# lajoiepy/cslam

Hardware: AMD Instinct MI355X
Metric: keyframes/sec (extract+match) on 100kx4096-D bank (higher is better)
Workload: dtype f32

## Files before the change

### cslam_amd/_lib.py

```python
import ctypes as C
import os
import subprocess

_HERE = os.path.dirname(os.path.abspath(__file__))
LIB_PATH = os.environ.get("CSLAM_HIP_LIB") or os.path.join(_HERE, "libcslam_hip.so")
CSRC_DIR = os.path.join(_HERE, "csrc")

F32, F64 = 0, 1
MODE_AUTO, MODE_SCAN, MODE_MFMA = 0, 1, 2


class CslamHipError(RuntimeError):
    pass


class CslamGraphError(CslamHipError):
    """CSLAM_E_GRAPH: the graph admits no Fiedler pair (not connected, singular junction Laplacian, TraceMIN breakdown) --
    the condition under which the reference's networkx call raises and acm.py:436-466 re-draws its start point.  Not a
    failure of the GPU path."""


class CslamUnsupportedError(CslamHipError):
    """CSLAM_E_UNSUPPORTED: an optional run-time dependency (RCCL, rocBLAS / rocSOLVER) was not found on this host."""

# ... 129 lines not shown
                                                   _vp, _vp, _vp, _vp, _vp, _vp, _vp, _vp, _vp, _vp, _vp, _vp, _vp, _vp, _vp, _vp, _vp, _vp]),
    "cslam_stereo_dense_dev": (_i, [_vp, _vp, _vp, _vp, _i, _vp, _i, _i, _i, _i, _vp, _vp, _vp, _vp, _vp, _vp, _vp, _vp]),
    "cslam_cloud_keyframes_stereo_dev": (_i, [_vp, _vp, _i, _vp, _vp, _vp, _vp, _vp, _i, _i, _i, _i, _i, C.c_double, C.c_double,
                                              _vp, _vp, _vp, _vp, _vp, _vp, _vp, _vp, _vp, _vp, _vp]),
    "cslam_wino4_fused_c64_h_dev": (_i, [_vp, _vp, _vp, _vp, _i, _i, _i, _i, _i, _i, _vp, C.c_float, _vp, _vp, _vp]),
    "cslam_conv3x3_direct_h_dev": (_i, [_vp, _vp, _vp, _i, _i, _i, _i, _i, _i, _i, _vp, _f, _vp, _vp, _vp]),
    "cslam_conv3x3_direct_r_dev": (_i, [_vp, _vp, _vp, _i, _i, _i, _i, _i, _i, _i, _vp, C.c_float, _vp, _vp, _vp]),
    "cslam_conv3x3_direct_r2_dev": (_i, [_vp, _vp, _vp, _i, _i, _i, _i, _i, _i, _i, _vp, C.c_float, _vp, _vp, _vp]),
    "cslam_conv_stem_direct_h_dev": (_i, [_vp, _vp, _vp, _vp, C.c_float, _vp, _vp, C.c_float, _i, _i, _i, _i, _vp, _vp, _vp, _vp]),
    "cslam_wino4_stem_c64_h_dev": (_i, [_vp, _vp, _vp, _vp, C.c_float, _vp, _vp, _i, _i, _i, _i, _vp, C.c_float, _vp, _vp, _vp]),
    "cslam_debug_wfh_prof_dev": (_i, [_vp]),
    "cslam_conv3x3_c3_amax_dev": (_i, [_vp, _vp, _vp, _i, _i, _i, _i, _i, _vp, _vp, _vp]),
    "cslam_wino4_input_h2_dev": (_i, [_vp, _i, _i, _i, _i, _vp, _vp, _vp]),
    "cslam_wino_gemm_h2_dev": (_i, [_vp, _vp, _i64, _i, _i, _vp, _vp]),
    "cslam_wino4_chain_h2_dev": (_i, [_vp, _vp, _i, _i, _i, _i, _vp, C.c_float, _vp, C.c_float, C.c_float, _vp, _vp, _vp, _vp]),
    "cslam_wino_zgemm_h2_dev": (_i, [_vp, _vp, _i64, _i, _i, _vp, _vp]),
    "cslam_wino4_output_z_dev": (_i, [_vp, _vp, _i, _i, _i, _i, _i, _i, _vp, C.c_float, _vp, _vp, _vp]),
    "cslam_conv_igemm_h2_dev": (_i, [_vp, _vp, _vp, _vp, _i, _i, _i, _i, _i, _i, _i, _i, _i, _i, _vp, C.c_float, _vp, _vp, _vp]),
    "cslam_conv_stem_pool_igemm_h2_dev": (_i, [_vp, _vp, _vp, _i, _i, _i, _i, _i, _i, _i, _i, _vp, C.c_float, _vp, _vp, _vp]),
    "cslam_conv_igemm_h2p_dev": (_i, [_vp, _i, _vp, _vp, _vp, _vp, _i, _vp, _i, _i, _i, _i, _i, _i, _i, _i, _i, _i, _vp, C.c_float,
                                      C.c_float, C.c_float, _vp, _i, _vp, _vp, _vp]),
    "cslam_conv3x3_direct_r_pairs_dev": (_i, [_vp, _vp, _vp, _i, _i, _i, _i, _i, _vp, C.c_float, C.c_float, C.c_float, _vp, _vp, _vp, _vp]),
    "cslam_conv3x3_direct_hp_dev": (_i, [_vp, _vp, _vp, _vp, _i, _i, _i, _i, _i, _i, _i, C.c_float, _vp, _vp, _vp]),
    "cslam_conv3x3_direct_p_dev": (_i, [_vp, _i, _vp, _vp, _vp, _vp, _i, _vp, _i, _i, _i, _i, _i, _i, _vp, C.c_float, C.c_float, C.c_float,
                                        _vp, _i, _vp, _vp, _vp]),
    "cslam_comm_unique_id": (_i, [_vp]),
    "cslam_comm_init": (_i, [_i, _i, _vp, _i, C.POINTER(_vp)]),
    "cslam_comm_destroy": (_i, [_vp]),
    "cslam_comm_info": (_i, [_vp, C.POINTER(_i), C.POINTER(_i)]),
    "cslam_allgather_queries_dev": (_i, [_vp, _vp, _i64, _i64, _vp, _vp]),
# ... 73 lines not shown
```

### cslam_amd/csrc/wino_chain.hip

```cpp
#include "common.h"
#include "pairs.h"
#include <hip/hip_fp16.h>

typedef float cf4 __attribute__((ext_vector_type(4)));
typedef unsigned cu2 __attribute__((ext_vector_type(2)));
typedef unsigned cu4 __attribute__((ext_vector_type(4)));

__device__ __forceinline__ void wc_at4(const cf4 m0, const cf4 m1, const cf4 m2, const cf4 m3, const cf4 m4, const cf4 m5,
                                       cf4 &s0, cf4 &s1, cf4 &s2, cf4 &s3) {
    const cf4 a = m1 + m2, bq = m1 - m2, c = m3 + m4, e = m3 - m4;
    s0 = m0 + a + c;
    s1 = bq + 2.0f * e;
    s2 = a + 4.0f * c;
    s3 = bq + 8.0f * e + m5;
}
__device__ __forceinline__ void wc_bt4(cf4 &d0, cf4 &d1, cf4 &d2, cf4 &d3, cf4 &d4, cf4 &d5) {
    const cf4 r0 = 4.0f * d0 - 5.0f * d2 + d4;
    const cf4 r1 = -4.0f * (d1 + d2) + d3 + d4;
    const cf4 r2 = 4.0f * (d1 - d2) - d3 + d4;
    const cf4 r3 = 2.0f * (d3 - d1) - d2 + d4;
    const cf4 r4 = 2.0f * (d1 - d3) - d2 + d4;
    const cf4 r5 = 4.0f * d1 - 5.0f * d3 + d5;
    d0 = r0; d1 = r1; d2 = r2; d3 = r3; d4 = r4; d5 = r5;
}

#define WC_THREADS 128
#define WC_RING 9

struct WcArgs {
    const float *mb;
    __half *vb;
    unsigned moff, voff;
    float *rp;
    int64_t mplane, vplane, mrow, vrow;
    int H, TH, Wr, tj;
    float inv, sc;
    cf4 bv;
    cf4 clim;
    bool odd;
};

template <int CG, bool OUT, bool LOAD, bool IN>
__device__ __forceinline__ void wc_step(const WcArgs &a, const int r, cf4 (&m)[36], float &vmax) {
    if (OUT) {
        cf4 s[4][6];
#pragma unroll
        for (int j = 0; j < 6; ++j)
            wc_at4(m[j], m[6 + j], m[12 + j], m[18 + j], m[24 + j], m[30 + j], s[0][j], s[1][j], s[2][j], s[3][j]);
#pragma unroll
        for (int i = 0; i < 4; ++i) {
            cf4 o[4];
            wc_at4(s[i][0], s[i][1], s[i][2], s[i][3], s[i][4], s[i][5], o[0], o[1], o[2], o[3]);
            const int h = 4 * r + i;
            float *row = a.rp + ((h % WC_RING) * a.Wr + 4 * a.tj) * CG;
            const cf4 lim = h < a.H ? a.clim : (cf4)(0.0f);
#pragma unroll
            for (int j = 0; j < 4; ++j) {
                cf4 v = __builtin_elementwise_max(o[j] * a.inv + a.bv, (cf4)(0.0f));
                v = __builtin_elementwise_min(v, (cf4)(lim[j]));
                vmax = fmaxf(fmaxf(vmax, fmaxf(v.x, v.y)), fmaxf(v.z, v.w));
                *(cf4 *)(row + j * CG) = v;
            }
        }
    }
    __syncthreads();
    if (LOAD) {
        const float *p = a.mb + (r + 1) * a.mrow;
#pragma unroll
        for (int q = 0; q < 36; ++q) m[q] = __builtin_nontemporal_load((const cf4 *)(p + q * a.mplane + a.moff));
    }
    if (IN) {
        const int h0 = 4 * (r - 1) - 1, w0 = 4 * a.tj - 1;
        const int Hr = 4 * a.TH;
        cf4 d[6][6];
#pragma unroll
        for (int i = 0; i < 6; ++i) {
            const int hh = h0 + i;
            const float *row = a.rp + ((hh + WC_RING) % WC_RING) * a.Wr * CG;
#pragma unroll
            for (int j = 0; j < 6; ++j) {
                const int ww = w0 + j;
                const bool in = (hh >= 0) & (hh < Hr) & (ww >= 0) & (ww < a.Wr);
                cf4 v = *(const cf4 *)(row + (j == 0 ? max(ww, 0) : j == 5 ? min(ww, a.Wr - 1) : ww) * CG);
                asm("" : "+v"(v));
                d[i][j] = in ? v * a.sc : (cf4)(0.0f);
            }
        }
#pragma unroll
        for (int j = 0; j < 6; ++j) wc_bt4(d[0][j], d[1][j], d[2][j], d[3][j], d[4][j], d[5][j]);
#pragma unroll
        for (int i = 0; i < 6; ++i) wc_bt4(d[i][0], d[i][1], d[i][2], d[i][3], d[i][4], d[i][5]);
        __half *o = a.vb + (r - 1) * a.vrow;
#pragma unroll
        for (int i = 0; i < 6; ++i)
#pragma unroll
            for (int j = 0; j < 6; ++j) {
                const cf4 v = d[i][j];
                const __half2 h0v = __floats2half2_rn(v.x, v.y), h1v = __floats2half2_rn(v.z, v.w);
                const __half2 l0v = __floats2half2_rn(sub_half<0>(v.x, h0v), sub_half<1>(v.y, h0v));
                const __half2 l1v = __floats2half2_rn(sub_half<0>(v.z, h1v), sub_half<1>(v.w, h1v));
                cu2 hi, lo;
                hi.x = *(const unsigned *)&h0v; hi.y = *(const unsigned *)&h1v;
                lo.x = *(const unsigned *)&l0v; lo.y = *(const unsigned *)&l1v;
                const cu2 give = a.odd ? hi : lo;
                cu2 got;
                got.x = (unsigned)__builtin_amdgcn_mov_dpp((int)give.x, 0xB1, 0xF, 0xF, true);
                got.y = (unsigned)__builtin_amdgcn_mov_dpp((int)give.y, 0xB1, 0xF, 0xF, true);
                cu4 v16;
                if (a.odd) { v16.x = got.x; v16.y = got.y; v16.z = lo.x; v16.w = lo.y; }
                else { v16.x = hi.x; v16.y = hi.y; v16.z = got.x; v16.w = got.y; }
                __builtin_nontemporal_store(v16, (cu4 *)(o + (6 * i + j) * a.vplane + a.voff));
            }
    }
    __syncthreads();
}

template <int CG>
__global__ __launch_bounds__(WC_THREADS) void wino4_chain_h2_kernel(const float *__restrict__ M, const float *__restrict__ bias,
                                                                     int B, int H, int W, int C,
                                                                     const unsigned *__restrict__ vscale, float inv_su,
                                                                     const unsigned *__restrict__ amax_x, float wl1, float bmax,
                                                                     unsigned *__restrict__ amax_out,
                                                                     unsigned *__restrict__ bound_out, __half *__restrict__ V2) {
    extern __shared__ __attribute__((aligned(16))) float ring[];
    __shared__ unsigned wg_amax;
    constexpr int C4G = CG / 4;
    WcArgs a;
    a.H = H;
    a.TH = (H + 3) >> 2;
    const int TW = (W + 3) >> 2;
    a.Wr = 4 * TW;
    const int ncg = C / CG;
    const int b = blockIdx.x / ncg, cg = blockIdx.x - b * ncg;
    a.tj = threadIdx.x / C4G;
    const int c4 = threadIdx.x % C4G;
    const int c = cg * CG + 4 * c4;
    const int64_t T = (int64_t)B * a.TH * TW;
    const int64_t t0 = (int64_t)b * a.TH * TW;
    if (threadIdx.x == 0) wg_amax = 0u;

    a.inv = inv_su / scale_le_327_68(__uint_as_float(*vscale));
    const float bound = fmaf(__uint_as_float(*amax_x), wl1, bmax);
    a.sc = scale_le_327_68(bound);
    if (blockIdx.x == 0 && threadIdx.x == 0) *bound_out = __float_as_uint(bound);
    a.bv = bias ? *(const cf4 *)(bias + c) : (cf4)(0.0f);
#pragma unroll
    for (int j = 0; j < 4; ++j) a.clim[j] = 4 * a.tj + j < W ? __builtin_inff() : 0.0f;
    a.odd = threadIdx.x & 1;
    a.mplane = T * C;
    a.vplane = T * 2 * C;
    a.mrow = (int64_t)TW * C;
    a.vrow = (int64_t)TW * 2 * C;
    a.mb = M + t0 * C + cg * CG;
    a.vb = V2 + t0 * 2 * C + cg * 2 * CG;
    a.moff = a.tj * C + 4 * c4;
    a.voff = a.tj * 2 * C + (c4 >> 3) * 64 + (4 * c4 & 31) + (a.odd ? 32 - 4 : 0);
    a.rp = ring + 4 * c4;
    float vmax = 0.0f;

    cf4 m[36];
#pragma unroll
    for (int q = 0; q < 36; ++q) m[q] = __builtin_nontemporal_load((const cf4 *)(a.mb + q * a.mplane + a.moff));
    const int TH = a.TH;
    if (TH == 1) {
        wc_step<CG, true, false, false>(a, 0, m, vmax);
    } else {
        wc_step<CG, true, true, false>(a, 0, m, vmax);
#pragma unroll 1
        for (int r = 1; r < TH - 1; ++r) wc_step<CG, true, true, true>(a, r, m, vmax);
        wc_step<CG, true, false, true>(a, TH - 1, m, vmax);
    }
    wc_step<CG, false, false, true>(a, TH, m, vmax);
#pragma unroll
    for (int o = 32; o > 0; o >>= 1) vmax = fmaxf(vmax, __shfl_xor(vmax, o, 64));
    if ((threadIdx.x & 63) == 0) atomicMax(&wg_amax, __float_as_uint(vmax));
    __syncthreads();
    if (threadIdx.x == 0 && wg_amax > *(volatile unsigned *)amax_out) atomicMax(amax_out, wg_amax);
}

template <int CG>
static int wino4_chain_launch(const float *d_M, const float *d_bias, int B, int H, int W, int C, const unsigned *d_vscale,
                              float inv_su, const unsigned *d_amax_x, float wl1, float bmax, unsigned *d_amax_out,
                              unsigned *d_bound_out, void *d_V2, void *stream) {
    const size_t lds = (size_t)WC_RING * 4 * ((W + 3) / 4) * CG * sizeof(float);
    ARG_CHECK(lds <= 144 * 1024, "map too wide for the LDS ring");
    static DeviceOnce once;
    int dev;
    if (once.todo(&dev)) {
        HIP_TRY(hipFuncSetAttribute((const void *)wino4_chain_h2_kernel<CG>, hipFuncAttributeMaxDynamicSharedMemorySize, 144 * 1024));
        once.done(dev);
    }
    hipLaunchKernelGGL(wino4_chain_h2_kernel<CG>, dim3((unsigned)((int64_t)B * (C / CG))), dim3(((W + 3) / 4) * (CG / 4)), lds, (hipStream_t)stream,
                       d_M, d_bias, B, H, W, C, d_vscale, inv_su, d_amax_x, wl1, bmax, d_amax_out, d_bound_out, (__half *)d_V2);
    HIP_TRY(hipGetLastError());
    return CSLAM_OK;
}

CSLAM_API int cslam_wino4_chain_h2_dev(const float *d_M, const float *d_bias, int B, int H, int W, int C,
                                       const unsigned *d_vscale, float inv_su, const unsigned *d_amax_x, float wl1, float bmax,
                                       unsigned *d_amax_out, unsigned *d_bound_out, void *d_V2, void *stream) {
    PTR_DEVICE(d_M);
    ARG_CHECK(d_M && d_V2 && d_vscale && d_amax_x && d_amax_out && d_bound_out, "NULL argument");
    ARG_CHECK(B >= 1 && H >= 1 && W >= 1, "empty map");
    ARG_CHECK(C >= 32 && (C % 32) == 0, "C must be a multiple of 32");
    ARG_CHECK(inv_su > 0.0f && wl1 >= 0.0f && bmax >= 0.0f, "inv_su must be positive, wl1 and bmax non-negative");
    const int TW = (W + 3) / 4;
    ARG_CHECK(TW <= 16, "maps wider than 64 pixels stay on the separate transforms");
    ARG_CHECK((int64_t)B * (C / 32) < (1LL << 31), "too many frames for one launch");
    if (TW <= 4 && (C % 128) == 0)
        return wino4_chain_launch<128>(d_M, d_bias, B, H, W, C, d_vscale, inv_su, d_amax_x, wl1, bmax, d_amax_out, d_bound_out, d_V2, stream);
    if (TW <= 8 && (C % 64) == 0)
        return wino4_chain_launch<64>(d_M, d_bias, B, H, W, C, d_vscale, inv_su, d_amax_x, wl1, bmax, d_amax_out, d_bound_out, d_V2, stream);
    return wino4_chain_launch<32>(d_M, d_bias, B, H, W, C, d_vscale, inv_su, d_amax_x, wl1, bmax, d_amax_out, d_bound_out, d_V2, stream);
}
```

### cslam_amd/vpr/netvlad.py

```python
import os
import pickle
from os.path import isfile, join

import numpy as np
import torch
from torch import nn

from .. import _lib
from . import heads
from .backbones import vgg16_features_trunk
from .winograd import WinogradTrunk

IMAGENET_DEFAULT_MEAN = heads.IMAGENET_DEFAULT_MEAN
IMAGENET_DEFAULT_STD = heads.IMAGENET_DEFAULT_STD


def _share_dir():
    try:
        from ament_index_python.packages import get_package_share_directory
        return get_package_share_directory("cslam")
    except Exception:
        return ""


def _strip_module(state):
    return {k.replace(".module.", "."): v for k, v in state.items()}
# ... 123 lines not shown
        self.trunk = None
        self._online = self._online_trunk = None
        self._lanes = []
        cent = torch.randn((64, 512), generator=g)
        cent = cent / cent.norm(dim=1, keepdim=True) * 0.5
        w = 2.0 * 10.0 * cent
        self.pool.load(w, cent)
        din = 64 * 512
        comp = torch.randn((pca_dim, din), generator=g, dtype=torch.float32) / din ** 0.5
        self.pca_components = heads.padded_rows(pca_dim, din, self.device)
        self.pca_components.copy_(comp)
        self.pca_pairs = heads.pca_pair_weights(self.pca_components)
        self.pca_mean_proj = torch.zeros(pca_dim, dtype=torch.float32, device=self.device)
        self.pca_inv_scale = None

    @torch.no_grad()
    def compute_embeddings_device(self, frames_u8, backbone_dtype=None, _trunk=None):
        x = heads.preprocess(frames_u8.contiguous(), self.crop)
        if self.backbone_conv == 'direct' or (backbone_dtype is not None and backbone_dtype != torch.float32):
            x = x.contiguous(memory_format=torch.channels_last)
        if backbone_dtype is not None and backbone_dtype != torch.float32:
            with torch.autocast("cuda", dtype=backbone_dtype):
                f = self.encoder(x)
            f = f.float()
        elif self.backbone_conv in ('winograd', 'winograd2'):
            if _trunk is not None:
                f = _trunk(x)
            else:
                if self.trunk is None:
                    self.trunk = WinogradTrunk(self.encoder, min_in_channels=64,
                                               tile=4 if self.backbone_conv == 'winograd' else 2, forms=self.trunk_forms)
                    self.trunk.input_bound = heads.normalised_image_bound()
                f = self.trunk(x)
        else:
            f = self.encoder(x)
        if heads.vlad_pairs_fit(f, self.pool.centroids, self.pca_pairs):
            a2, _ = heads.vlad_aggregate_pairs(f, self.pool.conv_weight, self.pool.conv_bias, self.pool.centroids,
                                               self.pca_pairs[0].shape[0], heads.VLAD_BOUND)
            return heads.pca_project_from_pairs(a2, self.pca_components, self.pca_mean_proj, self.pca_inv_scale, self.pca_pairs,
                                                heads.VLAD_BOUND)
        v = self.pool(f)
        return heads.pca_project(v, self.pca_components, self.pca_mean_proj, self.pca_inv_scale, self.pca_pairs, heads.VLAD_BOUND)

    def compute_embeddings_batch_device(self, frames_u8, chunk=512, lanes=2):
        if lanes <= 1 or frames_u8.shape[0] <= chunk or self.backbone_conv not in ('winograd', 'winograd2'):
            outs = [self.compute_embeddings_device(frames_u8[s:s + chunk]) for s in range(0, int(frames_u8.shape[0]), chunk)]
            return outs[0] if len(outs) == 1 else torch.cat(outs)

        def lane_trunk(i):
            if i == 0 and self.trunk is not None:
                return self.trunk
            trunk = WinogradTrunk(self.encoder, min_in_channels=64, tile=4 if self.backbone_conv == 'winograd' else 2, forms=self.trunk_forms)
            trunk.input_bound = heads.normalised_image_bound()
            if i == 0:
                self.trunk = trunk
            return trunk
        return heads.extract_over_lanes(self._lanes, frames_u8, chunk, lanes, lane_trunk,
                                        lambda fr, trunk: self.compute_embeddings_device(fr, _trunk=trunk))

    def compute_embedding(self, keyframe):
        if not self.enable:
            return np.random.rand(128)
        keyframe = np.ascontiguousarray(keyframe)
        if self.use_graph and keyframe.dtype == np.uint8 and keyframe.ndim == 3:
            if self._online is None:
                if self.backbone_conv != 'direct':
                    self._online_trunk = WinogradTrunk(self.encoder, min_in_channels=64, tile=2)
                self._online = heads.OnlineGraph(
# ... 7 lines not shown
```

### cslam_amd/vpr/winograd.py

```python
import os

import torch
from torch import nn

from .. import _lib
from .conv_kernels import (PairAct, _amax_slot, _out, _po, _residual_like, conv3x3_direct_h, conv3x3_direct_hp,
                           conv3x3_direct_p, conv3x3_direct_r, conv3x3_direct_r2, conv3x3_direct_r_pairs, conv_igemm, conv_igemm_p,
                           conv_stem_direct_h, direct_p_fits, pairs_to_float, stem_pool_fits, wino_fused64, wino_fused64_h,
                           wino_stem64_h)
from .heads import _p, _stream
from .pair_weights import (direct_pair_weights, direct_r2_pair_weights, direct_r_pair_weights, fused64_pair_weights,
                           fused64_weights, igemm_pair_weights, out_bound, split16_pair_weights, split16_weights,
                           stem_direct_pair_weights, stem_pair_weights, wino_weights)


def _pair(v):
    return tuple(v) if isinstance(v, (tuple, list)) else (v, v)


_TUNED = {"done": False}


def use_tuned_gemms():
    if _TUNED["done"] or os.environ.get("CSLAM_TUNED_GEMM", "1") == "0" or not torch.cuda.is_available():
# ... 24 lines not shown


def _f4_fits(B, H, W):
    t4h, t4w = -(-H // 4), -(-W // 4)
    return B * t4h * t4w >= 512 and 16 * t4h * t4w <= 1.35 * H * W


def _pair_pipeline(ws, x, layers, slots, relu, pool, residual, amax_out):
    lib = _lib.load()
    B, Cin, H, W = x.shape
    T = B * -(-H // 4) * -(-W // 4)
    s = _stream(x)
    V2 = ws._buf("V", 36 * T * Cin, x.device)
    _lib.check(lib.cslam_wino4_input_h2_dev(_p(x), B, H, W, Cin, _p(slots[0:1]), _p(V2), s))
    vscale = slots[0:1]
    for j, (U2, bias, wl1, bmax) in enumerate(layers):
        Cout = U2[0].shape[1]
        M = ws._buf("M", 36 * T * Cout, x.device)
        _lib.check(lib.cslam_wino_gemm_h2_dev(_p(V2), _p(U2[0]), T, Cin, Cout, _p(M), s))
        if j + 1 < len(layers):
            bound = ws._buf("chain_bounds", len(layers), x.device)[j + 1:j + 2]
            V2 = ws._buf("V", 36 * T * Cout, x.device)
            _lib.check(lib.cslam_wino4_chain_h2_dev(_p(M), _po(bias), B, H, W, Cout, _p(vscale), float(U2[1]), _p(slots[j:j + 1]),
                                                    wl1, bmax, _p(slots[j + 1:j + 2]), _p(bound), _p(V2), s))
            vscale, Cin = bound, Cout
    y = _out(B, Cout, H, W, pool, x.device)
    _lib.check(lib.cslam_wino4_output_scaled_dev(_p(M), _po(bias), _po(_residual_like(residual, y)), B, H, W, Cout, int(relu),
                                                 int(pool), _p(vscale), float(U2[1]), _po(amax_out), _p(y), s))
    return y


def wino_conv3x3(ws, x, U, U4, bias, relu, pool=False, residual=None, U3=None, amax_in=None, amax_out=None, U2=None):
    lib = _lib.load()
    B, Cin, H, W = x.shape
    Cout = U.shape[2]
    assert residual is None or not pool
    four = U4 is not None and _f4_fits(B, H, W)
    ws.amax_written = four and amax_out is not None
    T = B * -(-H // 4) * -(-W // 4) if four else B * -(-H // 2) * -(-W // 2)
    s = _stream(x)
    slot = None
    if four and (U2 is not None or U3 is not None):
        slot = amax_in if amax_in is not None else _amax_slot(x, ws._buf("amax", 1, x.device))
    z = four and U2 is not None and residual is None and _z_form(Cin, Cout)
    if four and U2 is not None and not z:
        return _pair_pipeline(ws, x, [(U2, bias, None, None)], slot, relu, pool, residual, amax_out)
    inv_su = 1.0
    if z:
        V2 = ws._buf("V", 36 * T * Cin, x.device)
        M = ws._buf("M", 36 * T * Cout, x.device)
        _lib.check(lib.cslam_wino4_input_h2_dev(_p(x), B, H, W, Cin, _p(slot), _p(V2), s))
        _lib.check(lib.cslam_wino_zgemm_h2_dev(_p(V2), _p(U2[0]), T, Cin, Cout, _p(M), s))
        inv_su = U2[1]
    elif slot is not None:
        V3 = ws._buf("V", (36 * T * 3 * Cin + 1) // 2, x.device).view(torch.float16)[:36 * T * 3 * Cin].view(36, T, 3 * Cin)
        _lib.check(lib.cslam_wino4_input_h3_dev(_p(x), B, H, W, Cin, _p(slot), _p(V3), s))
        M = torch.bmm(V3, U3[0], out_dtype=torch.float32)
        inv_su = U3[1]
    else:
        n2, Uu, fin = (36, U4, lib.cslam_wino4_input_dev) if four else (16, U, lib.cslam_wino_input_dev)
        V = ws._buf("V", n2 * T * Cin, x.device).view(n2, T, Cin)
# ... 164 lines not shown

class _Step(object):
    __slots__ = ("kind", "module", "conv", "relu", "pool", "U", "U4", "U3", "U2", "Up", "Uph", "bias", "stem", "Wd", "Wr", "Wdr", "Wdr2", "wl1", "bmax")

    def __init__(self):
        for name in self.__slots__:
            setattr(self, name, None)
        self.kind, self.relu, self.pool = "torch", False, False


def _wants(st):
    return st.U3 is not None or st.U2 is not None or st.Uph is not None or st.Wd is not None


TRUNK_FORMS = {"conv_direct": 1, "conv_direct_r": True, "conv_direct_r2": True, "stem_direct": True, "wino_stem": True, "fused_h": True, "split16_min_cin": None,
               "wino_chain": True}
CHAIN_TILE_COLS = (5, 16)
FP32_GEMM_FORMS = {"split16_min_cin": 0, "fused_h": False, "wino_stem": False}


def _pool2_at(mods, i):
    p = mods[i] if i < len(mods) else None
    return (isinstance(p, nn.MaxPool2d) and p.kernel_size in (2, (2, 2)) and p.stride in (2, (2, 2))
            and p.padding in (0, (0, 0)) and not p.ceil_mode)


class WinogradTrunk(_Workspace):

    def __init__(self, encoder, min_in_channels=256, tile=2, fused64=None, split16_h3=False, forms=None):
        super().__init__()
        self.encoder = encoder
# ... 72 lines not shown
                    st.pool = True
                    i += 1
            else:
                st.kind, st.module = "torch", m
                i += 1
            self.steps.append(st)
        if self.forms["wino_stem"]:
            for a, b in zip(self.steps, self.steps[1:]):
                if (a.kind == "c3" and a.relu and a.conv.out_channels == 64 and b.kind == "wino" and b.Uph is not None
                        and b.relu and b.conv.out_channels == 64):
                    a.stem = stem_pair_weights(a.conv.weight)
                    if self.forms["stem_direct"]:
                        a.Wr = stem_direct_pair_weights(b.conv.weight)
        return self

    def _chain_len(self, k, B, H, W):
        if not (self.forms["wino_chain"] and _f4_fits(B, H, W) and CHAIN_TILE_COLS[0] <= -(-W // 4) <= CHAIN_TILE_COLS[1]):
            return 1
        pair = lambda st_: (st_.kind == "wino" and st_.U2 is not None and st_.Wd is None and st_.Up is None
                            and not _z_form(st_.conv.in_channels, st_.conv.out_channels))
        n = 1
        while (k + n < len(self.steps) and pair(self.steps[k + n - 1]) and pair(self.steps[k + n])
               and self.steps[k + n - 1].relu and not self.steps[k + n - 1].pool):
            n += 1
        return n

    def _want(self, slots, j):
        return slots[j:j + 1] if j < len(self.steps) and _wants(self.steps[j]) else None


    def _stem_pair(self, k, x, slots):
        st, (B, _, H, W) = self.steps[k], x.shape
        nxt = self.steps[k + 1] if st.stem is not None else None
        if nxt is None or not (B * -(-H // 16) * -(-W // 16) >= self.fused_min_blocks and not (nxt.pool and (H % 2 or W % 2))
                               and B * H * W * 64 < 2 ** 31):
            return None
        slot = slots[k:k + 1]
        if self.input_bound is not None:
            slot.fill_(float(self.input_bound))
        else:
# ... 51 lines not shown
    def _fused64(self, k, x, have, slots):
        st, (B, _, H, W) = self.steps[k], x.shape
        if st.Up is None or (st.pool and (H % 2 or W % 2)):
            return None
        bh, bw = (16, 16) if st.Up.shape[1] == 36 else (8, 16)
        if B * -(-H // bh) * -(-W // bw) * st.Up.shape[2] // 4 < self.fused_min_blocks:
            return None
        if st.Uph is None or x.numel() >= 2 ** 31:
            return wino_fused64(x, st.Up, st.bias, st.relu, st.pool), None, 0
        slot = _amax_slot(x, slots[k:k + 1], have)
        want = self._want(slots, k + 1)
        return wino_fused64_h(x, st.Uph, st.bias, st.relu, st.pool, slot, want), want is not None, 0

    def _winograd(self, k, x, have, slots):
        st = self.steps[k]
        n = self._chain_len(k, x.shape[0], x.shape[2], x.shape[3])
        if n == 1:
            want = self._want(slots, k + 1)
            y = wino_conv3x3(self, x, st.U, st.U4, st.bias, st.relu, st.pool, U3=st.U3, U2=st.U2,
                             amax_in=slots[k:k + 1] if have else None, amax_out=want)
            return y, want is not None and self.amax_written, 0
        _amax_slot(x, slots[k:k + 1], have)
        want = self._want(slots, k + n)
        chain = self.steps[k:k + n]
        y = _pair_pipeline(self, x, [(t.U2, t.bias, t.wl1, t.bmax) for t in chain], slots[k:k + n], chain[-1].relu, chain[-1].pool,
                           None, want)
        return y, want is not None, n - 1

    @torch.no_grad()
    def __call__(self, x):
        slots = have = None
        if any(_wants(st) for st in self.steps):
            slots = self._buf("amax_slots", len(self.steps) + 1, x.device)
            slots.zero_()
        k = 0
        while k < len(self.steps):
            st = self.steps[k]
            if st.kind == "c3":
                x = x.contiguous()
                x, have, ran = self._stem_pair(k, x, slots) or self._first_layer(k, x, slots)
            else:
# ... 11 lines not shown
```

### include/cslam_hip.h

```cpp
#ifndef CSLAM_HIP_H
#define CSLAM_HIP_H

#include <stdint.h>

#ifdef __cplusplus
extern "C" {
#endif

#define CSLAM_OK 0
#define CSLAM_E_INVALID (-1)
#define CSLAM_E_HIP (-2)
#define CSLAM_E_NOMEM (-3)
#define CSLAM_E_DIM (-4)
#define CSLAM_E_UNSUPPORTED (-5)
#define CSLAM_E_GRAPH (-6)
#define CSLAM_E_LIMIT (-7)

#define CSLAM_F32 0
#define CSLAM_F64 1

#define CSLAM_MODE_AUTO 0
#define CSLAM_MODE_SCAN 1
#define CSLAM_MODE_MFMA 2

// ... 291 lines not shown
int cslam_wino_output_dev(const float *d_M, const float *d_bias, const float *d_residual, int B, int H, int W,
                          int C, int relu, int pool, float *d_y, void *stream);
int cslam_wino4_input_dev(const float *d_x, int B, int H, int W, int C, float *d_V, void *stream);
int cslam_wino4_output_dev(const float *d_M, const float *d_bias, const float *d_residual, int B, int H, int W,
                           int C, int relu, int pool, float *d_y, void *stream);
int cslam_absmax_dev(const float *d_x, int64_t n, unsigned *d_slot, void *stream);
int cslam_wino4_output_scaled_dev(const float *d_M, const float *d_bias, const float *d_residual, int B, int H, int W,
                                  int C, int relu, int pool, const unsigned *d_amax, float inv_su, unsigned *d_amax_out,
                                  float *d_y, void *stream);
int cslam_wino4_input_h2_dev(const float *d_x, int B, int H, int W, int C, const unsigned *d_amax, void *d_V2,
                             void *stream);
int cslam_wino_gemm_h2_dev(const void *d_V2, const void *d_U2, int64_t T, int Cin, int Cout, float *d_M, void *stream);
int cslam_wino4_chain_h2_dev(const float *d_M, const float *d_bias, int B, int H, int W, int C, const unsigned *d_vscale,
                             float inv_su, const unsigned *d_amax_x, float wl1, float bmax, unsigned *d_amax_out,
                             unsigned *d_bound_out, void *d_V2, void *stream);
int cslam_wino_zgemm_h2_dev(const void *d_V2, const void *d_U2, int64_t T, int Cin, int Cout, float *d_Z, void *stream);
int cslam_wino4_output_z_dev(const float *d_Z, const float *d_bias, int B, int H, int W, int C, int relu, int pool,
                             const unsigned *d_amax, float inv_su, unsigned *d_amax_out, float *d_y, void *stream);

int cslam_wino4_fused_c64_h_dev(const float *d_x, const void *d_Uh, const float *d_bias, const float *d_residual, int B,
                                int H, int W, int Cout, int relu, int pool, const unsigned *d_amax, float inv_su,
                                unsigned *d_amax_out, float *d_y, void *stream);
int cslam_conv3x3_direct_h_dev(const float *d_x, const void *d_w2, const float *d_bias, int B, int H, int W, int Cin, int Cout,
                               int relu, int pool, const unsigned *d_amax, float inv_sw, unsigned *d_amax_out, float *d_y,
                               void *stream);
int cslam_conv3x3_c3_amax_dev(const float *d_x, const float *d_wt, const float *d_bias, int B, int H, int W, int Cout,
                              int relu, float *d_y, unsigned *d_amax_out, void *stream);

int cslam_wino4_stem_c64_h_dev(const float *d_x0, const void *d_w1, const float *d_b1, const float *d_sumw, float inv_sw,
                               const void *d_Uh, const float *d_bias, int B, int H, int W, int pool,
// ... 64 lines not shown
```

Baseline: 18980.

## Add whole-map and pooled Winograd chain links to fuse more conv layers

Extends the fused Winograd output-to-input chain kernel with two new modes. A 'map' mode handles small feature maps (at most 16 tiles) in one block without the row-walk ring. A 'pool' mode applies a 2x2 max-pool inside the chain so the next layer's input transform is produced directly. The trunk planner now builds chains across these links, which removes separate output, pool and input-transform kernels and their HBM round trips. Map mode is on by default only for the extractor; pool mode is off by default, and the map kernel uses a different launch size and more LDS.

```diff
diff --git a/cslam_amd/_lib.py b/cslam_amd/_lib.py
--- a/cslam_amd/_lib.py
+++ b/cslam_amd/_lib.py
@@ -167,6 +167,8 @@
     "cslam_wino4_input_h2_dev": (_i, [_vp, _i, _i, _i, _i, _vp, _vp, _vp]),
     "cslam_wino_gemm_h2_dev": (_i, [_vp, _vp, _i64, _i, _i, _vp, _vp]),
     "cslam_wino4_chain_h2_dev": (_i, [_vp, _vp, _i, _i, _i, _i, _vp, C.c_float, _vp, C.c_float, C.c_float, _vp, _vp, _vp, _vp]),
+    "cslam_wino4_chain_map_h2_dev": (_i, [_vp, _vp, _i, _i, _i, _i, _vp, C.c_float, _vp, C.c_float, C.c_float, _vp, _vp, _vp, _i, _vp]),
+    "cslam_wino4_chain_pool_h2_dev": (_i, [_vp, _vp, _i, _i, _i, _i, _vp, C.c_float, _vp, C.c_float, C.c_float, _vp, _vp, _vp, _vp]),
     "cslam_wino_zgemm_h2_dev": (_i, [_vp, _vp, _i64, _i, _i, _vp, _vp]),
     "cslam_wino4_output_z_dev": (_i, [_vp, _vp, _i, _i, _i, _i, _i, _i, _vp, C.c_float, _vp, _vp, _vp]),
     "cslam_conv_igemm_h2_dev": (_i, [_vp, _vp, _vp, _vp, _i, _i, _i, _i, _i, _i, _i, _i, _i, _i, _vp, C.c_float, _vp, _vp, _vp]),
diff --git a/cslam_amd/csrc/wino_chain.hip b/cslam_amd/csrc/wino_chain.hip
--- a/cslam_amd/csrc/wino_chain.hip
+++ b/cslam_amd/csrc/wino_chain.hip
@@ -26,6 +26,10 @@
 
 #define WC_THREADS 128
 #define WC_RING 9
+#define WC_POOL_RING 8
+
+enum { WC_WALK, WC_MAP, WC_POOL };
+__host__ __device__ constexpr int wc_ring(int mode) { return mode == WC_WALK ? WC_RING : mode == WC_POOL ? WC_POOL_RING : 0; }
 
 struct WcArgs {
     const float *mb;
@@ -34,94 +38,108 @@
     float *rp;
     int64_t mplane, vplane, mrow, vrow;
     int H, TH, Wr, tj;
+    int TWn;
     float inv, sc;
     cf4 bv;
     cf4 clim;
     bool odd;
 };
 
-template <int CG, bool OUT, bool LOAD, bool IN>
+template <int CG, int MODE>
+__device__ __forceinline__ void wc_out(const WcArgs &a, const int r, const cf4 (&m)[36], float &vmax) {
+    constexpr int RING = wc_ring(MODE);
+    cf4 s[4][6];
+    cf4 top[4];
+#pragma unroll
+    for (int j = 0; j < 6; ++j)
+        wc_at4(m[j], m[6 + j], m[12 + j], m[18 + j], m[24 + j], m[30 + j], s[0][j], s[1][j], s[2][j], s[3][j]);
+#pragma unroll
+    for (int i = 0; i < 4; ++i) {
+        cf4 o[4];
+        wc_at4(s[i][0], s[i][1], s[i][2], s[i][3], s[i][4], s[i][5], o[0], o[1], o[2], o[3]);
+        const int h = 4 * r + i;
+        float *row = a.rp + ((RING ? h % RING : h) * a.Wr + 4 * a.tj) * CG;
+        const cf4 lim = h < a.H ? a.clim : (cf4)(0.0f);
+#pragma unroll
+        for (int j = 0; j < 4; ++j) {
+            cf4 v = __builtin_elementwise_max(o[j] * a.inv + a.bv, (cf4)(0.0f));
+            v = __builtin_elementwise_min(v, (cf4)(lim[j]));
+            vmax = fmaxf(fmaxf(vmax, fmaxf(v.x, v.y)), fmaxf(v.z, v.w));
+            if (MODE != WC_POOL) *(cf4 *)(row + j * CG) = v;
+            else top[j] = (i & 1) ? __builtin_elementwise_max(top[j], v) : v;
+        }
+        if (MODE == WC_POOL && (i & 1)) {
+            float *prow = a.rp + (((2 * r + (i >> 1)) % RING) * a.Wr + 2 * a.tj) * CG;
+            *(cf4 *)prow = __builtin_elementwise_max(top[0], top[1]);
+            *(cf4 *)(prow + CG) = __builtin_elementwise_max(top[2], top[3]);
+        }
+    }
+}
+
+template <int CG, int MODE>
+__device__ __forceinline__ void wc_in(const WcArgs &a, const int tr, __half *o) {
+    constexpr int RING = wc_ring(MODE);
+    const int h0 = 4 * tr - 1, w0 = 4 * a.tj - 1;
+    const int Hr = (MODE == WC_POOL ? 2 : 4) * a.TH;
+    cf4 d[6][6];
+#pragma unroll
+    for (int i = 0; i < 6; ++i) {
+        const int hh = h0 + i;
+        const float *row = a.rp + (RING ? (hh + RING) % RING : min(max(hh, 0), Hr - 1)) * a.Wr * CG;
+#pragma unroll
+        for (int j = 0; j < 6; ++j) {
+            const int ww = w0 + j;
+            const bool in = (hh >= 0) & (hh < Hr) & (ww >= 0) & (ww < a.Wr);
+            cf4 v = *(const cf4 *)(row + (j == 0 ? max(ww, 0) : j == 5 || MODE == WC_POOL ? min(ww, a.Wr - 1) : ww) * CG);
+            asm("" : "+v"(v));
+            d[i][j] = in ? v * a.sc : (cf4)(0.0f);
+        }
+    }
+#pragma unroll
+    for (int j = 0; j < 6; ++j) wc_bt4(d[0][j], d[1][j], d[2][j], d[3][j], d[4][j], d[5][j]);
+#pragma unroll
+    for (int i = 0; i < 6; ++i) wc_bt4(d[i][0], d[i][1], d[i][2], d[i][3], d[i][4], d[i][5]);
+#pragma unroll
+    for (int i = 0; i < 6; ++i)
+#pragma unroll
+        for (int j = 0; j < 6; ++j) {
+            const cf4 v = d[i][j];
+            const __half2 h0v = __floats2half2_rn(v.x, v.y), h1v = __floats2half2_rn(v.z, v.w);
+            const __half2 l0v = __floats2half2_rn(sub_half<0>(v.x, h0v), sub_half<1>(v.y, h0v));
+            const __half2 l1v = __floats2half2_rn(sub_half<0>(v.z, h1v), sub_half<1>(v.w, h1v));
+            cu2 hi, lo;
+            hi.x = *(const unsigned *)&h0v; hi.y = *(const unsigned *)&h1v;
+            lo.x = *(const unsigned *)&l0v; lo.y = *(const unsigned *)&l1v;
+            const cu2 give = a.odd ? hi : lo;
+            cu2 got;
+            got.x = (unsigned)__builtin_amdgcn_mov_dpp((int)give.x, 0xB1, 0xF, 0xF, true);
+            got.y = (unsigned)__builtin_amdgcn_mov_dpp((int)give.y, 0xB1, 0xF, 0xF, true);
+            cu4 v16;
+            if (a.odd) { v16.x = got.x; v16.y = got.y; v16.z = lo.x; v16.w = lo.y; }
+            else { v16.x = hi.x; v16.y = hi.y; v16.z = got.x; v16.w = got.y; }
+            __builtin_nontemporal_store(v16, (cu4 *)(o + (6 * i + j) * a.vplane + a.voff));
+        }
+}
+
+template <int CG, int MODE, bool OUT, bool LOAD, bool IN>
 __device__ __forceinline__ void wc_step(const WcArgs &a, const int r, cf4 (&m)[36], float &vmax) {
-    if (OUT) {
-        cf4 s[4][6];
-#pragma unroll
-        for (int j = 0; j < 6; ++j)
-            wc_at4(m[j], m[6 + j], m[12 + j], m[18 + j], m[24 + j], m[30 + j], s[0][j], s[1][j], s[2][j], s[3][j]);
-#pragma unroll
-        for (int i = 0; i < 4; ++i) {
-            cf4 o[4];
-            wc_at4(s[i][0], s[i][1], s[i][2], s[i][3], s[i][4], s[i][5], o[0], o[1], o[2], o[3]);
-            const int h = 4 * r + i;
-            float *row = a.rp + ((h % WC_RING) * a.Wr + 4 * a.tj) * CG;
-            const cf4 lim = h < a.H ? a.clim : (cf4)(0.0f);
-#pragma unroll
-            for (int j = 0; j < 4; ++j) {
-                cf4 v = __builtin_elementwise_max(o[j] * a.inv + a.bv, (cf4)(0.0f));
-                v = __builtin_elementwise_min(v, (cf4)(lim[j]));
-                vmax = fmaxf(fmaxf(vmax, fmaxf(v.x, v.y)), fmaxf(v.z, v.w));
-                *(cf4 *)(row + j * CG) = v;
-            }
-        }
-    }
+    if (OUT) wc_out<CG, MODE>(a, r, m, vmax);
     __syncthreads();
     if (LOAD) {
         const float *p = a.mb + (r + 1) * a.mrow;
 #pragma unroll
         for (int q = 0; q < 36; ++q) m[q] = __builtin_nontemporal_load((const cf4 *)(p + q * a.mplane + a.moff));
     }
-    if (IN) {
-        const int h0 = 4 * (r - 1) - 1, w0 = 4 * a.tj - 1;
-        const int Hr = 4 * a.TH;
-        cf4 d[6][6];
-#pragma unroll
-        for (int i = 0; i < 6; ++i) {
-            const int hh = h0 + i;
-            const float *row = a.rp + ((hh + WC_RING) % WC_RING) * a.Wr * CG;
-#pragma unroll
-            for (int j = 0; j < 6; ++j) {
-                const int ww = w0 + j;
-                const bool in = (hh >= 0) & (hh < Hr) & (ww >= 0) & (ww < a.Wr);
-                cf4 v = *(const cf4 *)(row + (j == 0 ? max(ww, 0) : j == 5 ? min(ww, a.Wr - 1) : ww) * CG);
-                asm("" : "+v"(v));
-                d[i][j] = in ? v * a.sc : (cf4)(0.0f);
-            }
-        }
-#pragma unroll
-        for (int j = 0; j < 6; ++j) wc_bt4(d[0][j], d[1][j], d[2][j], d[3][j], d[4][j], d[5][j]);
-#pragma unroll
-        for (int i = 0; i < 6; ++i) wc_bt4(d[i][0], d[i][1], d[i][2], d[i][3], d[i][4], d[i][5]);
-        __half *o = a.vb + (r - 1) * a.vrow;
-#pragma unroll
-        for (int i = 0; i < 6; ++i)
-#pragma unroll
-            for (int j = 0; j < 6; ++j) {
-                const cf4 v = d[i][j];
-                const __half2 h0v = __floats2half2_rn(v.x, v.y), h1v = __floats2half2_rn(v.z, v.w);
-                const __half2 l0v = __floats2half2_rn(sub_half<0>(v.x, h0v), sub_half<1>(v.y, h0v));
-                const __half2 l1v = __floats2half2_rn(sub_half<0>(v.z, h1v), sub_half<1>(v.w, h1v));
-                cu2 hi, lo;
-                hi.x = *(const unsigned *)&h0v; hi.y = *(const unsigned *)&h1v;
-                lo.x = *(const unsigned *)&l0v; lo.y = *(const unsigned *)&l1v;
-                const cu2 give = a.odd ? hi : lo;
-                cu2 got;
-                got.x = (unsigned)__builtin_amdgcn_mov_dpp((int)give.x, 0xB1, 0xF, 0xF, true);
-                got.y = (unsigned)__builtin_amdgcn_mov_dpp((int)give.y, 0xB1, 0xF, 0xF, true);
-                cu4 v16;
-                if (a.odd) { v16.x = got.x; v16.y = got.y; v16.z = lo.x; v16.w = lo.y; }
-                else { v16.x = hi.x; v16.y = hi.y; v16.z = got.x; v16.w = got.y; }
-                __builtin_nontemporal_store(v16, (cu4 *)(o + (6 * i + j) * a.vplane + a.voff));
-            }
-    }
+    if (IN && MODE != WC_POOL) wc_in<CG, MODE>(a, r - 1, a.vb + (r - 1) * a.vrow);
+    if (IN && MODE == WC_POOL && !(r & 1) && r >= 2 && a.tj < a.TWn) wc_in<CG, MODE>(a, (r >> 1) - 1, a.vb + ((r >> 1) - 1) * a.vrow);
     __syncthreads();
 }
 
-template <int CG>
-__global__ __launch_bounds__(WC_THREADS) void wino4_chain_h2_kernel(const float *__restrict__ M, const float *__restrict__ bias,
-                                                                     int B, int H, int W, int C,
-                                                                     const unsigned *__restrict__ vscale, float inv_su,
-                                                                     const unsigned *__restrict__ amax_x, float wl1, float bmax,
-                                                                     unsigned *__restrict__ amax_out,
-                                                                     unsigned *__restrict__ bound_out, __half *__restrict__ V2) {
+template <int CG, int MODE>
+__device__ __forceinline__ void wc_kernel(const float *__restrict__ M, const float *__restrict__ bias, int B, int H, int W, int C,
+                                          const unsigned *__restrict__ vscale, float inv_su, const unsigned *__restrict__ amax_x,
+                                          float wl1, float bmax, unsigned *__restrict__ amax_out, unsigned *__restrict__ bound_out,
+                                          __half *__restrict__ V2) {
     extern __shared__ __attribute__((aligned(16))) float ring[];
     __shared__ unsigned wg_amax;
     constexpr int C4G = CG / 4;
@@ -129,14 +147,18 @@
     a.H = H;
     a.TH = (H + 3) >> 2;
     const int TW = (W + 3) >> 2;
-    a.Wr = 4 * TW;
+    a.Wr = (MODE == WC_POOL ? 2 : 4) * TW;
+    const int THn = MODE == WC_POOL ? ((H >> 1) + 3) >> 2 : a.TH;
+    a.TWn = MODE == WC_POOL ? ((W >> 1) + 3) >> 2 : TW;
     const int ncg = C / CG;
     const int b = blockIdx.x / ncg, cg = blockIdx.x - b * ncg;
-    a.tj = threadIdx.x / C4G;
+    const int tile = threadIdx.x / C4G;
+    const int ti = MODE == WC_MAP ? tile / TW : 0;
+    a.tj = tile - ti * TW;
     const int c4 = threadIdx.x % C4G;
     const int c = cg * CG + 4 * c4;
-    const int64_t T = (int64_t)B * a.TH * TW;
-    const int64_t t0 = (int64_t)b * a.TH * TW;
+    const int64_t T = (int64_t)B * a.TH * TW, Tn = (int64_t)B * THn * a.TWn;
+    const int64_t t0 = (int64_t)b * a.TH * TW, t0n = (int64_t)b * THn * a.TWn;
     if (threadIdx.x == 0) wg_amax = 0u;
 
     a.inv = inv_su / scale_le_327_68(__uint_as_float(*vscale));
@@ -148,13 +170,13 @@
     for (int j = 0; j < 4; ++j) a.clim[j] = 4 * a.tj + j < W ? __builtin_inff() : 0.0f;
     a.odd = threadIdx.x & 1;
     a.mplane = T * C;
-    a.vplane = T * 2 * C;
+    a.vplane = Tn * 2 * C;
     a.mrow = (int64_t)TW * C;
-    a.vrow = (int64_t)TW * 2 * C;
+    a.vrow = (int64_t)a.TWn * 2 * C;
     a.mb = M + t0 * C + cg * CG;
-    a.vb = V2 + t0 * 2 * C + cg * 2 * CG;
-    a.moff = a.tj * C + 4 * c4;
-    a.voff = a.tj * 2 * C + (c4 >> 3) * 64 + (4 * c4 & 31) + (a.odd ? 32 - 4 : 0);
+    a.vb = V2 + t0n * 2 * C + cg * 2 * CG;
+    a.moff = tile * C + 4 * c4;
+    a.voff = tile * 2 * C + (c4 >> 3) * 64 + (4 * c4 & 31) + (a.odd ? 32 - 4 : 0);
     a.rp = ring + 4 * c4;
     float vmax = 0.0f;
 
@@ -162,15 +184,26 @@
 #pragma unroll
     for (int q = 0; q < 36; ++q) m[q] = __builtin_nontemporal_load((const cf4 *)(a.mb + q * a.mplane + a.moff));
     const int TH = a.TH;
-    if (TH == 1) {
-        wc_step<CG, true, false, false>(a, 0, m, vmax);
+    if (MODE == WC_MAP) {
+        wc_out<CG, MODE>(a, ti, m, vmax);
+        __syncthreads();
+        wc_in<CG, MODE>(a, ti, a.vb);
     } else {
-        wc_step<CG, true, true, false>(a, 0, m, vmax);
+        if (TH == 1) {
+            wc_step<CG, MODE, true, false, false>(a, 0, m, vmax);
+        } else {
+            wc_step<CG, MODE, true, true, false>(a, 0, m, vmax);
 #pragma unroll 1
-        for (int r = 1; r < TH - 1; ++r) wc_step<CG, true, true, true>(a, r, m, vmax);
-        wc_step<CG, true, false, true>(a, TH - 1, m, vmax);
-    }
-    wc_step<CG, false, false, true>(a, TH, m, vmax);
+            for (int r = 1; r < TH - 1; ++r) wc_step<CG, MODE, true, true, true>(a, r, m, vmax);
+            wc_step<CG, MODE, true, false, true>(a, TH - 1, m, vmax);
+        }
+        if (MODE == WC_WALK) {
+            wc_step<CG, MODE, false, false, true>(a, TH, m, vmax);
+        } else {
+#pragma unroll 1
+            for (int r = TH; r <= 2 * THn; ++r) wc_step<CG, MODE, false, false, true>(a, r, m, vmax);
+        }
+    }
 #pragma unroll
     for (int o = 32; o > 0; o >>= 1) vmax = fmaxf(vmax, __shfl_xor(vmax, o, 64));
     if ((threadIdx.x & 63) == 0) atomicMax(&wg_amax, __float_as_uint(vmax));
@@ -178,38 +211,84 @@
     if (threadIdx.x == 0 && wg_amax > *(volatile unsigned *)amax_out) atomicMax(amax_out, wg_amax);
 }
 
+#define WC_PARAMS const float *__restrict__ M, const float *__restrict__ bias, int B, int H, int W, int C,                                   \
+                  const unsigned *__restrict__ vscale, float inv_su, const unsigned *__restrict__ amax_x, float wl1, float bmax,           \
+                  unsigned *__restrict__ amax_out, unsigned *__restrict__ bound_out, __half *__restrict__ V2
+#define WC_PASS M, bias, B, H, W, C, vscale, inv_su, amax_x, wl1, bmax, amax_out, bound_out, V2
+
 template <int CG>
+__global__ __launch_bounds__(WC_THREADS) void wino4_chain_h2_kernel(WC_PARAMS) { wc_kernel<CG, WC_WALK>(WC_PASS); }
+
+template <int CG>
+__global__ __launch_bounds__(WC_THREADS) void wino4_chain_pool_h2_kernel(WC_PARAMS) { wc_kernel<CG, WC_POOL>(WC_PASS); }
+
+template <int CG>
+__global__ __launch_bounds__(4 * CG, 2) void wino4_chain_map_h2_kernel(WC_PARAMS) { wc_kernel<CG, WC_MAP>(WC_PASS); }
+
+template <int CG, int MODE>
 static int wino4_chain_launch(const float *d_M, const float *d_bias, int B, int H, int W, int C, const unsigned *d_vscale,
                               float inv_su, const unsigned *d_amax_x, float wl1, float bmax, unsigned *d_amax_out,
                               unsigned *d_bound_out, void *d_V2, void *stream) {
-    const size_t lds = (size_t)WC_RING * 4 * ((W + 3) / 4) * CG * sizeof(float);
+    const int TH = (H + 3) / 4, TW = (W + 3) / 4;
+    const size_t lds = (size_t)(MODE == WC_MAP ? 4 * TH : wc_ring(MODE)) * (MODE == WC_POOL ? 2 : 4) * TW * CG * sizeof(float);
     ARG_CHECK(lds <= 144 * 1024, "map too wide for the LDS ring");
+    const auto kernel = MODE == WC_MAP ? wino4_chain_map_h2_kernel<CG> : MODE == WC_POOL ? wino4_chain_pool_h2_kernel<CG> : wino4_chain_h2_kernel<CG>;
     static DeviceOnce once;
     int dev;
     if (once.todo(&dev)) {
-        HIP_TRY(hipFuncSetAttribute((const void *)wino4_chain_h2_kernel<CG>, hipFuncAttributeMaxDynamicSharedMemorySize, 144 * 1024));
+        HIP_TRY(hipFuncSetAttribute((const void *)kernel, hipFuncAttributeMaxDynamicSharedMemorySize, 144 * 1024));
         once.done(dev);
     }
-    hipLaunchKernelGGL(wino4_chain_h2_kernel<CG>, dim3((unsigned)((int64_t)B * (C / CG))), dim3(((W + 3) / 4) * (CG / 4)), lds, (hipStream_t)stream,
+    hipLaunchKernelGGL(kernel, dim3((unsigned)((int64_t)B * (C / CG))), dim3((MODE == WC_MAP ? TH : 1) * TW * (CG / 4)), lds, (hipStream_t)stream,
                        d_M, d_bias, B, H, W, C, d_vscale, inv_su, d_amax_x, wl1, bmax, d_amax_out, d_bound_out, (__half *)d_V2);
     HIP_TRY(hipGetLastError());
     return CSLAM_OK;
 }
 
+#define WC_CHECK_COMMON                                                                                                                     \
+    PTR_DEVICE(d_M);                                                                                                                        \
+    ARG_CHECK(d_M && d_V2 && d_vscale && d_amax_x && d_amax_out && d_bound_out, "NULL argument");                                           \
+    ARG_CHECK(B >= 1 && H >= 1 && W >= 1, "empty map");                                                                                     \
+    ARG_CHECK(C >= 32 && (C % 32) == 0, "C must be a multiple of 32");                                                                      \
+    ARG_CHECK(inv_su > 0.0f && wl1 >= 0.0f && bmax >= 0.0f, "inv_su must be positive, wl1 and bmax non-negative");                          \
+    ARG_CHECK((int64_t)B * (C / 32) < (1LL << 31), "too many frames for one launch")
+#define WC_LAUNCH_ARGS d_M, d_bias, B, H, W, C, d_vscale, inv_su, d_amax_x, wl1, bmax, d_amax_out, d_bound_out, d_V2, stream
+
+template <int MODE>
+static int wino4_chain_walk(const float *d_M, const float *d_bias, int B, int H, int W, int C, const unsigned *d_vscale, float inv_su,
+                            const unsigned *d_amax_x, float wl1, float bmax, unsigned *d_amax_out, unsigned *d_bound_out, void *d_V2,
+                            void *stream) {
+    const int TW = (W + 3) / 4;
+    ARG_CHECK(TW <= 16, "maps wider than 64 pixels stay on the separate transforms");
+    if (TW <= 4 && (C % 128) == 0) return wino4_chain_launch<128, MODE>(WC_LAUNCH_ARGS);
+    if (TW <= 8 && (C % 64) == 0) return wino4_chain_launch<64, MODE>(WC_LAUNCH_ARGS);
+    return wino4_chain_launch<32, MODE>(WC_LAUNCH_ARGS);
+}
+
 CSLAM_API int cslam_wino4_chain_h2_dev(const float *d_M, const float *d_bias, int B, int H, int W, int C,
                                        const unsigned *d_vscale, float inv_su, const unsigned *d_amax_x, float wl1, float bmax,
                                        unsigned *d_amax_out, unsigned *d_bound_out, void *d_V2, void *stream) {
-    PTR_DEVICE(d_M);
-    ARG_CHECK(d_M && d_V2 && d_vscale && d_amax_x && d_amax_out && d_bound_out, "NULL argument");
-    ARG_CHECK(B >= 1 && H >= 1 && W >= 1, "empty map");
-    ARG_CHECK(C >= 32 && (C % 32) == 0, "C must be a multiple of 32");
-    ARG_CHECK(inv_su > 0.0f && wl1 >= 0.0f && bmax >= 0.0f, "inv_su must be positive, wl1 and bmax non-negative");
-    const int TW = (W + 3) / 4;
-    ARG_CHECK(TW <= 16, "maps wider than 64 pixels stay on the separate transforms");
-    ARG_CHECK((int64_t)B * (C / 32) < (1LL << 31), "too many frames for one launch");
-    if (TW <= 4 && (C % 128) == 0)
-        return wino4_chain_launch<128>(d_M, d_bias, B, H, W, C, d_vscale, inv_su, d_amax_x, wl1, bmax, d_amax_out, d_bound_out, d_V2, stream);
-    if (TW <= 8 && (C % 64) == 0)
-        return wino4_chain_launch<64>(d_M, d_bias, B, H, W, C, d_vscale, inv_su, d_amax_x, wl1, bmax, d_amax_out, d_bound_out, d_V2, stream);
-    return wino4_chain_launch<32>(d_M, d_bias, B, H, W, C, d_vscale, inv_su, d_amax_x, wl1, bmax, d_amax_out, d_bound_out, d_V2, stream);
-}
+    WC_CHECK_COMMON;
+    return wino4_chain_walk<WC_WALK>(WC_LAUNCH_ARGS);
+}
+
+CSLAM_API int cslam_wino4_chain_pool_h2_dev(const float *d_M, const float *d_bias, int B, int H, int W, int C,
+                                            const unsigned *d_vscale, float inv_su, const unsigned *d_amax_x, float wl1, float bmax,
+                                            unsigned *d_amax_out, unsigned *d_bound_out, void *d_V2, void *stream) {
+    WC_CHECK_COMMON;
+    ARG_CHECK((H % 2) == 0 && (W % 2) == 0, "H and W must be even: other maps stay on the separate transforms");
+    return wino4_chain_walk<WC_POOL>(WC_LAUNCH_ARGS);
+}
+
+CSLAM_API int cslam_wino4_chain_map_h2_dev(const float *d_M, const float *d_bias, int B, int H, int W, int C,
+                                           const unsigned *d_vscale, float inv_su, const unsigned *d_amax_x, float wl1, float bmax,
+                                           unsigned *d_amax_out, unsigned *d_bound_out, void *d_V2, int group, void *stream) {
+    WC_CHECK_COMMON;
+    ARG_CHECK(((H + 3) / 4) * ((W + 3) / 4) <= 16, "maps of more than 16 tiles stay on the tile-row walk");
+    ARG_CHECK(group == 0 || group == 32 || group == 64 || group == 128, "group must be 0, 32, 64 or 128");
+    if (group == 0) group = (C % 64) == 0 ? 64 : 32;
+    ARG_CHECK((C % group) == 0, "C must be a multiple of the channel group");
+    if (group == 128) return wino4_chain_launch<128, WC_MAP>(WC_LAUNCH_ARGS);
+    if (group == 64) return wino4_chain_launch<64, WC_MAP>(WC_LAUNCH_ARGS);
+    return wino4_chain_launch<32, WC_MAP>(WC_LAUNCH_ARGS);
+}
diff --git a/cslam_amd/vpr/netvlad.py b/cslam_amd/vpr/netvlad.py
--- a/cslam_amd/vpr/netvlad.py
+++ b/cslam_amd/vpr/netvlad.py
@@ -9,7 +9,7 @@
 from .. import _lib
 from . import heads
 from .backbones import vgg16_features_trunk
-from .winograd import WinogradTrunk
+from .winograd import EXTRACTOR_FORMS, WinogradTrunk
 
 IMAGENET_DEFAULT_MEAN = heads.IMAGENET_DEFAULT_MEAN
 IMAGENET_DEFAULT_STD = heads.IMAGENET_DEFAULT_STD
@@ -163,6 +163,12 @@
         self.pca_mean_proj = torch.zeros(pca_dim, dtype=torch.float32, device=self.device)
         self.pca_inv_scale = None
 
+    def _batch_trunk(self):
+        trunk = WinogradTrunk(self.encoder, min_in_channels=64, tile=4 if self.backbone_conv == 'winograd' else 2,
+                              forms=EXTRACTOR_FORMS if self.trunk_forms is None else self.trunk_forms)
+        trunk.input_bound = heads.normalised_image_bound()
+        return trunk
+
     @torch.no_grad()
     def compute_embeddings_device(self, frames_u8, backbone_dtype=None, _trunk=None):
         x = heads.preprocess(frames_u8.contiguous(), self.crop)
@@ -177,9 +183,7 @@
                 f = _trunk(x)
             else:
                 if self.trunk is None:
-                    self.trunk = WinogradTrunk(self.encoder, min_in_channels=64,
-                                               tile=4 if self.backbone_conv == 'winograd' else 2, forms=self.trunk_forms)
-                    self.trunk.input_bound = heads.normalised_image_bound()
+                    self.trunk = self._batch_trunk()
                 f = self.trunk(x)
         else:
             f = self.encoder(x)
@@ -199,8 +203,7 @@
         def lane_trunk(i):
             if i == 0 and self.trunk is not None:
                 return self.trunk
-            trunk = WinogradTrunk(self.encoder, min_in_channels=64, tile=4 if self.backbone_conv == 'winograd' else 2, forms=self.trunk_forms)
-            trunk.input_bound = heads.normalised_image_bound()
+            trunk = self._batch_trunk()
             if i == 0:
                 self.trunk = trunk
             return trunk
diff --git a/cslam_amd/vpr/winograd.py b/cslam_amd/vpr/winograd.py
--- a/cslam_amd/vpr/winograd.py
+++ b/cslam_amd/vpr/winograd.py
@@ -62,16 +62,24 @@
     V2 = ws._buf("V", 36 * T * Cin, x.device)
     _lib.check(lib.cslam_wino4_input_h2_dev(_p(x), B, H, W, Cin, _p(slots[0:1]), _p(V2), s))
     vscale = slots[0:1]
-    for j, (U2, bias, wl1, bmax) in enumerate(layers):
+    for j, (U2, bias, wl1, bmax, link) in enumerate(layers):
         Cout = U2[0].shape[1]
         M = ws._buf("M", 36 * T * Cout, x.device)
         _lib.check(lib.cslam_wino_gemm_h2_dev(_p(V2), _p(U2[0]), T, Cin, Cout, _p(M), s))
-        if j + 1 < len(layers):
+        if link is not None:
             bound = ws._buf("chain_bounds", len(layers), x.device)[j + 1:j + 2]
-            V2 = ws._buf("V", 36 * T * Cout, x.device)
-            _lib.check(lib.cslam_wino4_chain_h2_dev(_p(M), _po(bias), B, H, W, Cout, _p(vscale), float(U2[1]), _p(slots[j:j + 1]),
-                                                    wl1, bmax, _p(slots[j + 1:j + 2]), _p(bound), _p(V2), s))
-            vscale, Cin = bound, Cout
+            Hn, Wn = (H // 2, W // 2) if link == "pool" else (H, W)
+            Tn = B * -(-Hn // 4) * -(-Wn // 4)
+            V2 = ws._buf("V", 36 * Tn * Cout, x.device)
+            args = (_p(M), _po(bias), B, H, W, Cout, _p(vscale), float(U2[1]), _p(slots[j:j + 1]), wl1, bmax, _p(slots[j + 1:j + 2]),
+                    _p(bound), _p(V2))
+            if link == "map":
+                _lib.check(lib.cslam_wino4_chain_map_h2_dev(*args, 0, s))
+            elif link == "pool":
+                _lib.check(lib.cslam_wino4_chain_pool_h2_dev(*args, s))
+            else:
+                _lib.check(lib.cslam_wino4_chain_h2_dev(*args, s))
+            vscale, Cin, H, W, T = bound, Cout, Hn, Wn, Tn
     y = _out(B, Cout, H, W, pool, x.device)
     _lib.check(lib.cslam_wino4_output_scaled_dev(_p(M), _po(bias), _po(_residual_like(residual, y)), B, H, W, Cout, int(relu),
                                                  int(pool), _p(vscale), float(U2[1]), _po(amax_out), _p(y), s))
@@ -92,7 +100,7 @@
         slot = amax_in if amax_in is not None else _amax_slot(x, ws._buf("amax", 1, x.device))
     z = four and U2 is not None and residual is None and _z_form(Cin, Cout)
     if four and U2 is not None and not z:
-        return _pair_pipeline(ws, x, [(U2, bias, None, None)], slot, relu, pool, residual, amax_out)
+        return _pair_pipeline(ws, x, [(U2, bias, None, None, None)], slot, relu, pool, residual, amax_out)
     inv_su = 1.0
     if z:
         V2 = ws._buf("V", 36 * T * Cin, x.device)
@@ -287,7 +295,8 @@
 
 
 TRUNK_FORMS = {"conv_direct": 1, "conv_direct_r": True, "conv_direct_r2": True, "stem_direct": True, "wino_stem": True, "fused_h": True, "split16_min_cin": None,
-               "wino_chain": True}
+               "wino_chain": True, "wino_chain_map": False, "wino_chain_pool": False}
+EXTRACTOR_FORMS = {"wino_chain_map": True}
 CHAIN_TILE_COLS = (5, 16)
 FP32_GEMM_FORMS = {"split16_min_cin": 0, "fused_h": False, "wino_stem": False}
 
@@ -390,16 +399,28 @@
                         a.Wr = stem_direct_pair_weights(b.conv.weight)
         return self
 
-    def _chain_len(self, k, B, H, W):
-        if not (self.forms["wino_chain"] and _f4_fits(B, H, W) and CHAIN_TILE_COLS[0] <= -(-W // 4) <= CHAIN_TILE_COLS[1]):
-            return 1
+    def _chain_links(self, k, B, H, W):
         pair = lambda st_: (st_.kind == "wino" and st_.U2 is not None and st_.Wd is None and st_.Up is None
                             and not _z_form(st_.conv.in_channels, st_.conv.out_channels))
-        n = 1
-        while (k + n < len(self.steps) and pair(self.steps[k + n - 1]) and pair(self.steps[k + n])
-               and self.steps[k + n - 1].relu and not self.steps[k + n - 1].pool):
-            n += 1
-        return n
+        links = []
+        while _f4_fits(B, H, W) and k + 1 < len(self.steps) and pair(self.steps[k]) and pair(self.steps[k + 1]) and self.steps[k].relu:
+            th, tw = -(-H // 4), -(-W // 4)
+            if self.steps[k].pool:
+                fits = H % 2 == 0 and W % 2 == 0 and tw <= 16 and _f4_fits(B, H // 2, W // 2)
+                link = "pool" if self.forms["wino_chain_pool"] and fits else None
+                H, W = H // 2, W // 2
+            elif self.forms["wino_chain_map"] and th * tw <= 16:
+                link = "map"
+            else:
+                link = "walk" if self.forms["wino_chain"] and CHAIN_TILE_COLS[0] <= tw <= CHAIN_TILE_COLS[1] else None
+            if link is None:
+                break
+            links.append(link)
+            k += 1
+        return links
+
+    def _chain_len(self, k, B, H, W):
+        return len(self._chain_links(k, B, H, W)) + 1
 
     def _want(self, slots, j):
         return slots[j:j + 1] if j < len(self.steps) and _wants(self.steps[j]) else None
@@ -481,7 +502,8 @@
 
     def _winograd(self, k, x, have, slots):
         st = self.steps[k]
-        n = self._chain_len(k, x.shape[0], x.shape[2], x.shape[3])
+        links = self._chain_links(k, x.shape[0], x.shape[2], x.shape[3])
+        n = len(links) + 1
         if n == 1:
             want = self._want(slots, k + 1)
             y = wino_conv3x3(self, x, st.U, st.U4, st.bias, st.relu, st.pool, U3=st.U3, U2=st.U2,
@@ -490,8 +512,8 @@
         _amax_slot(x, slots[k:k + 1], have)
         want = self._want(slots, k + n)
         chain = self.steps[k:k + n]
-        y = _pair_pipeline(self, x, [(t.U2, t.bias, t.wl1, t.bmax) for t in chain], slots[k:k + n], chain[-1].relu, chain[-1].pool,
-                           None, want)
+        y = _pair_pipeline(self, x, [(t.U2, t.bias, t.wl1, t.bmax, link) for t, link in zip(chain, links + [None])], slots[k:k + n],
+                           chain[-1].relu, chain[-1].pool, None, want)
         return y, want is not None, n - 1
 
     @torch.no_grad()
diff --git a/include/cslam_hip.h b/include/cslam_hip.h
--- a/include/cslam_hip.h
+++ b/include/cslam_hip.h
@@ -329,6 +329,12 @@
 int cslam_wino4_chain_h2_dev(const float *d_M, const float *d_bias, int B, int H, int W, int C, const unsigned *d_vscale,
                              float inv_su, const unsigned *d_amax_x, float wl1, float bmax, unsigned *d_amax_out,
                              unsigned *d_bound_out, void *d_V2, void *stream);
+int cslam_wino4_chain_map_h2_dev(const float *d_M, const float *d_bias, int B, int H, int W, int C, const unsigned *d_vscale,
+                                 float inv_su, const unsigned *d_amax_x, float wl1, float bmax, unsigned *d_amax_out,
+                                 unsigned *d_bound_out, void *d_V2, int group, void *stream);
+int cslam_wino4_chain_pool_h2_dev(const float *d_M, const float *d_bias, int B, int H, int W, int C, const unsigned *d_vscale,
+                                  float inv_su, const unsigned *d_amax_x, float wl1, float bmax, unsigned *d_amax_out,
+                                  unsigned *d_bound_out, void *d_V2, void *stream);
 int cslam_wino_zgemm_h2_dev(const void *d_V2, const void *d_U2, int64_t T, int Cin, int Cout, float *d_Z, void *stream);
 int cslam_wino4_output_z_dev(const float *d_Z, const float *d_bias, int B, int H, int W, int C, int relu, int pool,
                              const unsigned *d_amax, float inv_su, unsigned *d_amax_out, float *d_y, void *stream);
```

Result: no change. 19100 (median of 6 runs) (+0.7%).
